# jumerckx/Monodepth2.jl

Measured on AMD Instinct MI355X. Metric: train-step images/sec, ResNet-18 416×128; 1/2/4/8 MI355X + roofline %, higher is better.
Workload: dtype fp32; 1 GPU; train_step resnet18 depth+pose decoders, 4-scale photometric loss, ADAM; batch_per_gpu=12, global_batch=12, height=128, width=416, parallelism=dp1

## Files before the change

monodepth2.jl_amd/csrc/model.cpp:

```cpp
#include "model.h"
#include "head.h"
#include "testmode.h"

#include <algorithm>
#include <cmath>
#include <cstring>

namespace md2 {

namespace {

struct PConv {
  int cin = 0, cout = 0, k = 1, stride = 1, pad = 0, reflect = 0;
  bool bias = false;
  long w = -1, b = -1;
};
struct PBN {
  int c = 0;
  long g = -1, b = -1;
};
struct BlockSpec {
  std::vector<PConv> convs;
  std::vector<PBN> bns;
  bool down = false;
// ... 600 lines not shown
      MD2_TRY(alloc(&pose_rep, 2L * ND * 6));
      MD2_TRY(alloc(&d_pose_rep, 2L * ND * 6));
      if (cfg.automask) MD2_TRY(alloc(&amask_rep, (long)ND * cfg.H * cfg.W));
    }
    tail.N = ND;
    tail.C = C;
    tail.W = cfg.W;
    tail.H = cfg.H;
    tail.nscales = A.nlevels;
    int li = 0;
    for (auto& d : br)
      if (d.head >= 0) {
        tail.dw[li] = 2 * d.w;
        tail.dh[li] = 2 * d.h;
        tail.smooth_w[li] = cfg.smoothness * cfg.scales[li];
        ++li;
      }
    tail.divisor = (float)A.nlevels;
    tail.smooth_normalize = 1;
    std::memcpy(tail.K, cfg.K, sizeof(tail.K));
    std::memcpy(tail.invK, cfg.invK, sizeof(tail.invK));
    tail.min_depth = cfg.min_depth;
    tail.max_depth = cfg.max_depth;
    tail.x_frame_stride = (long)C * cfg.H * cfg.W;
    tail.x_sample_stride = E > 0 ? 0 : 3 * tail.x_frame_stride;
    tail.target = cfg.target;
    tail.src0 = cfg.src0;
    tail.src1 = cfg.src1;
    tail.invert_mask = (cfg.src0 < cfg.target ? 1 : 0) | (cfg.src1 < cfg.target ? 2 : 0);
    tail.sigmoid_grad = 1;
    {
      float* q;
      MD2_TRY(alloc(&q, loss_tail_workspace_bytes(tail) / sizeof(float) + 64));
      tail_ws = q;
    }
    MD2_TRY(alloc(&loss_buf, 16));
    if (cfg.automask) MD2_TRY(alloc(&amask, (long)N * cfg.H * cfg.W));
    return build_pack_table();
  }

  struct ProfRec {
    hipEvent_t a, b;
    int cat;
    double work;
    char tag[64];
  };
  bool prof = false;
  std::vector<ProfRec> recs;
  std::vector<hipEvent_t> evpool;
  size_t evi = 0;
  hipEvent_t ev() {
    if (evi == evpool.size()) {
      hipEvent_t e;
      (void)hipEventCreate(&e);
      evpool.push_back(e);
    }
    return evpool[evi++];
  }
  hipEvent_t prof_begin(hipStream_t st) {
    if (!prof) return nullptr;
    hipEvent_t e = ev();
    (void)hipEventRecord(e, st);
    return e;
  }
  void prof_end(hipEvent_t a, int cat, double work, hipStream_t st, const char* pass = nullptr,
                const ConvShape* s = nullptr) {
    if (!prof) return;
    hipEvent_t b = ev();
    (void)hipEventRecord(b, st);
    ProfRec r{a, b, cat, work, {0}};
    if (pass && s) {
      const int ar = conv_last_arith();
      snprintf(r.tag, sizeof(r.tag), "%s %dx%d/%d%s %d->%d %dx%d n%d [%s]", pass, s->KH, s->KW, s->stride,
               s->reflect ? "r" : "", s->Cin, s->Cout, s->H, s->W, s->N,
               ar == 6 ? "bf16x6" : ar == 1 ? "fp32" : "valu");
    }
    else if (pass)
      snprintf(r.tag, sizeof(r.tag), "%s", pass);
    recs.push_back(r);
  }
  static double conv_flops(const ConvShape& s) {
    return 2.0 * s.N * (double)s.Ho * s.Wo * s.Cout * weight_cin(s) * s.KH * s.KW;
  }

  int conv_f(RConv& c, int nimg, const TensorIn& in, float* out, long out_bs, int act,
             int accumulate, hipStream_t st) {
    ConvShape s = c.s;
    s.N = nimg;
    TensorOut o;
    o.p0 = out;
    o.bs0 = out_bs;
    o.bias = P(c.p.b);
    o.act = act;
    o.accumulate = accumulate;
    hipEvent_t e = prof_begin(st);
    MD2_TRY(conv_fwd(s, in, c.wpf, o, ws_conv(), st));
    prof_end(e, c.cat, conv_flops(s), st, "fwd", &s);
    return MD2_OK;
  }
  int conv_f_bn(RConv& c, int nimg, const TensorIn& in, float* y, long out_bs, RBN& bn, long HW,
                hipStream_t st, int slot = 0) {
    ConvShape s = c.s;
    s.N = nimg;
    TensorOut o;
    o.p0 = y;
    o.bs0 = out_bs;
    o.bias = P(c.p.b);
    SplitKDefer d;
    BNStatsWs wst = bn_ws(bn, nimg, HW, slot);
    if (fuse_bnstats) d.stats = wst.partials;
    d.keep_reduce = !fuse_splitk;
    hipEvent_t e = prof_begin(st);
    MD2_TRY(conv_fwd(s, in, c.wpf, o, ws_conv(), st, fuse_splitk || fuse_bnstats ? &d : nullptr));
    if (d.stats_parts > 0) {
      if (bn_collapse) {
        MD2_CHECK_ARG(bn.p.c <= 4096, "conv_f_bn: BN channels");
        double* col = bn_collapsed + (long)slot * 2 * 4096;
        MD2_TRY(bn_partials_collapse(wst.partials, bn.p.c, d.stats_parts, col, st));
        bn.part = col;
        bn.parts = 1;
      } else {
        bn.part = wst.partials;
        bn.parts = d.stats_parts;
      }
      prof_end(e, c.cat, conv_flops(s), st, "fwd", &s);
      return MD2_OK;
    }
    if (d.splits > 0) {
      BNStatsWs w = bn_ws(bn, nimg, HW, slot);
      MD2_TRY(bn_stats_partial_slabs(SlabIn{d.slab, d.splits}, y, nimg, bn.p.c, HW, w, st));
      prof_end(e, c.cat, conv_flops(s), st, "fwd", &s);
      return MD2_OK;
    }
    prof_end(e, c.cat, conv_flops(s), st, "fwd", &s);
    return bn_fwd(bn, y, nimg, HW, st, slot);
  }
  const bool fuse_skip_bwd = [] {
    const char* v = getenv("MD2_FUSE_SKIP_BWD");
    return !(v && v[0] == '0');
  }();
  const bool fuse_pool_fwd = [] {
    const char* v = getenv("MD2_FUSE_POOL_FWD");
    return !(v && v[0] == '0');
  }();
  const bool fuse_pool_bwd = [] {
    const char* v = getenv("MD2_FUSE_POOL_BWD");
    return !(v && v[0] == '0');
  }();
  const bool bn_collapse = tuning_knob("MD2_BN_COLLAPSE", 0) != 0;
  const bool fuse_bnstats = [] {
    const char* v = getenv("MD2_FUSE_BNSTATS");
    return !(v && v[0] == '0');
  }();
  const bool fuse_splitk = [] {
    const char* v = getenv("MD2_FUSE_SPLITK");
    return !(v && v[0] == '0');
  }();
  static TensorIn tin(const float* p, int C, long HW) {
    TensorIn t;
    t.p0 = p;
    t.c0 = C;
    t.bs0 = (long)C * HW;
    return t;
  }

  PackJob* pack_jobs = nullptr;
  int pack_njobs = 0;
  long pack_blocks = 0;

  int build_pack_table() {
    std::vector<PackJob> jobs;
    auto pk = [&](RConv& c) { jobs.push_back(conv_pack_job(c.s, params + c.p.w, c.wpf, c.wpd)); };
    pk(stem);
    for (auto& sg : stages)
      for (auto& b : sg) {
        for (auto& e : b.st) pk(e.conv);
        if (b.down) pk(b.dconv);
      }
    for (auto& d : br) {
      pk(d.c1);
      pk(d.c2);
      if (d.head >= 0) pk(d.hc);
    }
    pk(sq);
    pk(p1);
    pk(p2);
    long blocks = 0;
    for (auto& j : jobs) {
      j.block_begin = blocks;
      blocks += conv_pack_job_blocks(j);
    }
    void* q = nullptr;
    MD2_HIP(hipMalloc(&q, jobs.size() * sizeof(PackJob)));
    allocs.push_back(q);
    MD2_HIP(hipMemcpy(q, jobs.data(), jobs.size() * sizeof(PackJob), hipMemcpyHostToDevice));
    pack_jobs = (PackJob*)q;
    pack_njobs = (int)jobs.size();
    pack_blocks = blocks;
    for (int k = 0; k < 6; ++k) {
      long b0, e0;
      segment_range(k, b0, e0);
      std::vector<PackJob> sj;
      long sb = 0;
      for (PackJob j : jobs) {
        const long off = (long)(j.w - params);
        if (off < b0 || off >= e0) continue;
        j.block_begin = sb;
        sb += conv_pack_job_blocks(j);
        sj.push_back(j);
      }
      seg_pack[k] = SegPack{};
      if (sj.empty()) continue;
      void* qs = nullptr;
      MD2_HIP(hipMalloc(&qs, sj.size() * sizeof(PackJob)));
      allocs.push_back(qs);
      MD2_HIP(hipMemcpy(qs, sj.data(), sj.size() * sizeof(PackJob), hipMemcpyHostToDevice));
      seg_pack[k] = SegPack{(PackJob*)qs, (int)sj.size(), sb};
    }
    return MD2_OK;
  }

  void segment_range(int k, long& b, long& e) const {
    const ArchSpec& S = spec;
    switch (k) {
      case 0: b = S.depth_begin; e = S.total; break;
      case 1: b = S.stage_begin[4]; e = S.depth_begin; break;
      case 2: b = S.stage_begin[3]; e = S.stage_begin[4]; break;
      case 3: b = S.stage_begin[2]; e = S.stage_begin[3]; break;
      case 4: b = S.stage_begin[1]; e = S.stage_begin[2]; break;
      default: b = 0; e = S.stage_begin[1]; break;
    }
  }

  int adam_segment(int k, float* am, float* av, float lr, float b1, float b2, float eps, float bc1,
                   float bc2, float gscale, hipStream_t st) {
    long b0, e0;
    segment_range(k, b0, e0);
    MD2_HIP(hipEventRecord(seg_ev, st));
    MD2_HIP(hipStreamWaitEvent(upd, seg_ev, 0));
    MD2_TRY(adam_step(params + b0, grads + b0, am + b0, av + b0, e0 - b0, lr, b1, b2, eps, bc1, bc2,
                      gscale, upd));
    if (seg_pack[k].njobs) MD2_TRY(conv_pack_batch(seg_pack[k].jobs, seg_pack[k].njobs, seg_pack[k].blocks, upd));
    MD2_HIP(hipEventRecord(upd_ev, upd));
    upd_recorded = true;
    return MD2_OK;
  }
  int adam_join(hipStream_t st) {
    if (upd_recorded) MD2_HIP(hipStreamWaitEvent(st, upd_ev, 0));
    return MD2_OK;
  }

  int repack(hipStream_t st) { return conv_pack_batch(pack_jobs, pack_njobs, pack_blocks, st); }

  BNStatsWs bn_ws(RBN& bn, int nimg, long HW, int slot) {
    BNStatsWs w = bnws;
    w.partials += slot * bn_slot;
    w.parts = bn_parts(bn.p.c, nimg, HW);
    bn.part = w.partials;
    bn.parts = w.parts;
    return w;
  }
  int bn_fwd(RBN& bn, const float* y, int nimg, long HW, hipStream_t st, int slot = 0) {
    return bn_stats_partial(y, nimg, bn.p.c, HW, bn_ws(bn, nimg, HW, slot), st);
  }
  BNStatsIn bn_in(const RBN& bn) {
    BNStatsIn s;
    s.part = bn.part;
    s.parts = bn.parts;
    s.gamma = P(bn.p.g);
    s.beta = P(bn.p.b);
    s.mean = bn.mean;
    s.invstd = bn.invstd;
    s.run_mean = bn.rmean;
    s.run_var = bn.rvar;
    return s;
  }

  bool testmode = false;
  float* wfold = nullptr;
  float* tm_st = nullptr;
  FoldJob* fold_jobs = nullptr;
  int fold_njobs = 0;
  long fold_blocks = 0;
  PackJob* tm_pack_jobs = nullptr;
  int tm_pack_njobs = 0;
  long tm_pack_blocks = 0;

  int testmode_alloc() {
    if (wfold) return MD2_OK;
    MD2_TRY(alloc(&wfold, spec.depth_begin));
    MD2_TRY(alloc(&tm_st, bn_layout.off[bn_layout.n]));
    std::vector<FoldJob> fj;
    std::vector<PackJob> pj;
    int k = 0;
    auto job = [&](RConv* c, RBN& bn) -> int {
      bn.ts = tm_st + bn_layout.off[k++];
      bn.tt = bn.ts + bn.p.c;
      FoldJob j;
      j.gamma = P(bn.p.g); j.beta = P(bn.p.b);
      j.mean = bn.rmean; j.var = bn.rvar;
      j.s = bn.ts; j.t = bn.tt;
      j.Cout = bn.p.c;
      if (c) {
        const long per = (long)c->p.cin * c->p.k * c->p.k;
        MD2_CHECK_ARG(per % 4 == 0 && c->p.cout == bn.p.c, "test mode: conv weight rows of 4n floats");
        j.w = params + c->p.w;
// ... 254 lines not shown
    MD2_TRY(conv_f(p2, 2 * N, tin(pc1, 256, hw4), pc2, 256 * hw4, ACT_RELU, 0, st));
    return pose_head_fwd(pc2, 2 * N, 256, hw4, P(spec.p3.w), P(spec.p3.b), means, pose, st);
  }

  int forward(const float* x, hipStream_t st) {
    const long fs = (long)cfg.arch.in_ch * cfg.H * cfg.W;
    TensorIn in;
    in.p0 = x;
    in.c0 = cfg.arch.in_ch;
    in.bdiv = N;
    in.bs0 = 3 * fs;
    in.bhi = fs;
    MD2_TRY(encoder(in, B, st));
    if (pose_overlap()) {
      MD2_TRY(stream_wait(st, side, fork_ev));
      MD2_TRY(pose_fwd(side));
      MD2_TRY(decoder_fwd(N, T0, st));
      MD2_TRY(stream_wait(side, st, join_ev));
    } else {
      MD2_TRY(decoder_fwd(N, T0, st));
      MD2_TRY(pose_fwd(st));
    }
    return MD2_OK;
  }

  int forward_loss(const float* x, const float* automask, float* loss, float* terms,
                   hipStream_t st) {
    MD2_TRY(forward(x, st));
    const float* disps[MAX_SCALES] = {};
    LossTailOut o{};
    int li = 0;
    for (auto& d : br)
      if (d.head >= 0) {
        disps[li] = d.disp;
        o.d_disp[li] = d.d_head;
        ++li;
      }
    o.loss = loss ? loss : loss_buf;
    o.terms = terms;
    o.d_pose = E > 0 ? d_pose_rep : d_pose;
    hipEvent_t pev[2 * MAX_SCALES] = {};
    if (prof) {
      for (int k = 0; k < 2; ++k) pev[k] = ev();
      o.photo_events = pev;
    }
    if (cfg.automask && !automask) {
      MD2_TRY(launch_automask(x, tail.x_sample_stride, tail.x_frame_stride, tail.target, tail.src0,
                              tail.src1, N, cfg.arch.in_ch, cfg.H, cfg.W, amask, st));
      automask = amask;
    }
    const float* tail_pose = pose;
    if (E > 0) {
      MD2_TRY(repeat_rows(pose, 2L * N, 6, NP, pose_rep, st));
      tail_pose = pose_rep;
      if (cfg.automask) {
        MD2_TRY(repeat_rows(automask, N, cfg.H * cfg.W, NP, amask_rep, st));
        automask = amask_rep;
      }
    }
    MD2_TRY(loss_tail_run(tail, disps, tail_pose, x, cfg.automask ? automask : nullptr, 1.f, o, tail_ws, st));
    if (E > 0) MD2_TRY(repeat_rows_adjoint(d_pose_rep, 2L * N, 6, NP, d_pose, st));
    if (prof) {
      const double bytes = (double)tail.nscales * ND * cfg.H * cfg.W * (8.0 + 12.0 * cfg.arch.in_ch);
      recs.push_back({pev[0], pev[1], PROF_PHOTO, bytes, "photometric (all scales)"});
    }
    return MD2_OK;
  }

  int profile_records(int max, double* ms, double* work, int* cat, char* tags, int tag_len,
                      int* count) {
    int k = 0;
    for (auto& r : recs) {
      if (k >= max) break;
      MD2_HIP(hipEventSynchronize(r.b));
      float t = 0.f;
      MD2_HIP(hipEventElapsedTime(&t, r.a, r.b));
      ms[k] = t;
      work[k] = r.work;
      cat[k] = r.cat;
      if (tags && tag_len > 0) {
        strncpy(tags + (long)k * tag_len, r.tag, tag_len - 1);
        tags[(long)k * tag_len + tag_len - 1] = 0;
      }
      ++k;
    }
    *count = k;
    recs.clear();
    evi = 0;
    return MD2_OK;
  }

  int profile_read(double* out, int ncat) {
    for (int c = 0; c < ncat * 3; ++c) out[c] = 0.0;
    for (auto& r : recs) {
      MD2_HIP(hipEventSynchronize(r.b));
      float ms = 0.f;
      MD2_HIP(hipEventElapsedTime(&ms, r.a, r.b));
      if (r.cat < ncat) {
        out[r.cat * 3 + 0] += ms;
        out[r.cat * 3 + 1] += r.work;
        out[r.cat * 3 + 2] += 1.0;
      }
    }
    recs.clear();
    evi = 0;
    return MD2_OK;
  }

  int conv_w(RConv& c, int nimg, const TensorIn& in, const float* dy, hipStream_t st) {
    ConvShape s = c.s;
    s.N = nimg;
    hipEvent_t e = prof_begin(st);
    MD2_TRY(conv_wgrad(s, in, dy, grads + c.p.w, Gd(c.p.b), 0, ws_conv(), st, c.p.b >= 0 ? bp_pending : nullptr,
                       bp_parts));
    bp_pending = nullptr;
    prof_end(e, c.cat, conv_flops(s), st, "wgrad", &s);
    return MD2_OK;
  }
  int conv_wd(RConv& c, int nimg, const TensorIn& in, const float* dy, float* dx, long dx_bs,
              int acc, hipStream_t st, float* dx1 = nullptr, long dx1_bs = 0, int c0 = 1 << 30) {
    MD2_TRY(conv_w(c, nimg, in, dy, st));
    return conv_d(c, nimg, dy, dx, dx_bs, acc, st, dx1, dx1_bs, c0);
  }
  int conv_d(RConv& c, int nimg, const float* dy, float* dx, long dx_bs, int acc, hipStream_t st,
             float* dx1 = nullptr, long dx1_bs = 0, int c0 = 1 << 30) {
    ConvShape s = c.s;
    s.N = nimg;
    TensorOut o;
    o.p0 = dx;
    o.bs0 = dx_bs;
    o.p1 = dx1;
    o.bs1 = dx1_bs;
    o.c0 = c0;
    o.accumulate = acc;
    hipEvent_t e = prof_begin(st);
    MD2_TRY(conv_dgrad(s, dy, c.wpd, o, ws_conv(), st));
    prof_end(e, c.cat, conv_flops(s), st, "dgrad", &s);
    return MD2_OK;
  }
  int conv_d_bn(RConv& c, int nimg, const float* dy, float* da, long da_bs, RBN& bn, const float* y,
                long HW, float* dyprev, hipStream_t st) {
    ConvShape s = c.s;
    s.N = nimg;
    TensorOut o;
    o.p0 = da;
    o.bs0 = da_bs;
    SplitKDefer d;
    hipEvent_t e = prof_begin(st);
    MD2_TRY(conv_dgrad(s, dy, c.wpd, o, ws_conv(), st, fuse_splitk ? &d : nullptr));
    if (d.splits == 0) {
      prof_end(e, c.cat, conv_flops(s), st, "dgrad", &s);
      return bn_bwd(bn, da, nullptr, y, nimg, HW, dyprev, nullptr, 0, st, true);
    }
    BNStatsWs w = bnws;
    w.parts = bn_parts(bn.p.c, nimg, HW);
    MD2_TRY(bn_bwd_partial_slabs(SlabIn{d.slab, d.splits}, da, y, bn.mean, bn.invstd, nimg, bn.p.c,
                                 HW, w, st, P(bn.p.g), P(bn.p.b)));
    prof_end(e, c.cat, conv_flops(s), st, "dgrad", &s);
    return bn_bwd_apply_fused(da, nullptr, y, bn.mean, bn.invstd, P(bn.p.g), w, Gd(bn.p.g),
                              Gd(bn.p.b), nimg, bn.p.c, HW, dyprev, nullptr, 0, st, P(bn.p.b));
  }
  float* bp_ws = nullptr;
  const float* bp_pending = nullptr;
  int bp_parts = 0;
  int act_bias(const float* out, const float* dout, float* dpre, int nimg, int C, long HW, int act,
               hipStream_t st, float* bp_buf = nullptr) {
    if (HW % 4 != 0 || (long)C * act_bias_parts(C, nimg, HW) > BP_WS) {
      bp_pending = nullptr;
      return act_backward(out, dout, dpre, (long)nimg * C * HW, act, st);
    }
    float* bp = bp_buf ? bp_buf : ws_bp();
    MD2_TRY(act_backward_bias(out, dout, dpre, nimg, C, HW, act, bp, st));
    bp_pending = bp;
    bp_parts = act_bias_parts(C, nimg, HW);
    return MD2_OK;
  }
  static constexpr long BP_WS = 8192;

  int bn_bwd(RBN& bn, const float* dout, const float* mask, const float* y, int nimg, long HW,
             float* dy, float* dres, int dres_acc, hipStream_t st, bool relu_from_y = false,
             SkipAdd sk = SkipAdd{}, int slot = 0) {
    BNStatsWs w = bnws;
    w.partials += slot * bn_slot;
    w.parts = bn_parts(bn.p.c, nimg, HW);
    const float* mg = relu_from_y ? P(bn.p.g) : nullptr;
    const float* mb = relu_from_y ? P(bn.p.b) : nullptr;
    if (relu_from_y) mask = nullptr;
    MD2_TRY(bn_bwd_partial(dout, mask, y, bn.mean, bn.invstd, nimg, bn.p.c, HW, w, st, mg, mb, sk));
    return bn_bwd_apply_fused(dout, mask, y, bn.mean, bn.invstd, P(bn.p.g), w, Gd(bn.p.g),
                              Gd(bn.p.b), nimg, bn.p.c, HW, dy, dres, dres_acc, st, mb, sk);
  }
  bool skip_fused(int si) const {
    return fuse_skip_bwd && si >= 1 && si <= 3 && d_skip[si] && ((long)featH[si] * featW[si]) % 4 == 0;
  }
  SkipAdd skip_add(int si) const {
    SkipAdd sk;
    if (!skip_fused(si)) return sk;
    const long fsz = (long)featC[si] * featH[si] * featW[si];
    sk.skip = d_skip[si];
    sk.lo = (long)T0 * fsz;
    sk.hi = (long)(T0 + N) * fsz;
    return sk;
  }

  int block_bwd(EncBlock& b, hipStream_t st, SkipAdd sk = SkipAdd{}, bool eov = false) {
    const int nimg = B;
    const long ohw = (long)b.H * b.W, ihw = (long)b.Hin * b.Win;
    const int ns = (int)b.st.size();
    EncStage& last = b.st.back();
    MD2_TRY(y_claim(ycur, st));
    MD2_TRY(bn_bwd(last.bn, b.d_out, last.a, last.y, nimg, ohw, ybuf(ycur), b.down ? G : b.d_in, 0, st,
                   false, sk));
    const bool dov = b.down && down_overlap();
    if (b.down) {
      hipStream_t sd = dov ? side : st;
      if (dov) MD2_TRY(stream_wait(st, side, fork_ev));
      MD2_TRY(bn_bwd(b.dbn, G, nullptr, b.yd, nimg, ohw, DYD, nullptr, 0, sd, false, SkipAdd{}, 1));
      side_ws = true;
      const int rc = conv_wd(b.dconv, nimg, tin(b.in, b.Cin, ihw), DYD, b.d_in, (long)b.Cin * ihw, 0, sd);
      side_ws = false;
      MD2_TRY(rc);
      if (dov) MD2_HIP(hipEventRecord(join_ev, side));
    }
    for (int k = ns - 1; k >= 0; --k) {
      EncStage& e = b.st[k];
      const float* xin = k == 0 ? b.in : b.st[k - 1].a;
      const int cin = e.conv.p.cin;
      const long hin = (long)e.conv.s.H * e.conv.s.W;
      float* dy = ybuf(ycur);
      const bool wmain = eov && k == 0 && enc_wgrad_main0;
      if (eov && !wmain) {
        MD2_TRY(stream_wait(st, side, fork_ev));
        side_ws = true;
        const int rc = conv_w(e.conv, nimg, tin(xin, cin, hin), dy, side);
        side_ws = false;
        MD2_TRY(rc);
        MD2_HIP(hipEventRecord(ev_y[ycur], side));
        y_pending[ycur] = true;
      } else if (!wmain) {
        MD2_TRY(conv_w(e.conv, nimg, tin(xin, cin, hin), dy, st));
      }
      if (k > 0) {
        EncStage& pe = b.st[k - 1];
        const int nx = ycur ^ 1;
        MD2_TRY(y_claim(nx, st));
        MD2_TRY(conv_d_bn(e.conv, nimg, dy, DA, (long)cin * hin, pe.bn, pe.y, hin, ybuf(nx), st));
        ycur = nx;
      } else {
        if (dov) MD2_HIP(hipStreamWaitEvent(st, join_ev, 0));
        MD2_TRY(conv_d(e.conv, nimg, dy, b.d_in, (long)cin * hin, 1, st));
        if (wmain) MD2_TRY(conv_w(e.conv, nimg, tin(xin, cin, hin), dy, st));
      }
    }
    return MD2_OK;
  }

  int pose_bwd(hipStream_t st) {
    side_ws = true;
    const int rc = pose_bwd_body(st);
    side_ws = false;
    return rc;
  }
  int pose_bwd_body(hipStream_t st) {
    const long hw4 = (long)featH[4] * featW[4];
    float* DP = DPRE_side;
    MD2_TRY(pose_head_bwd(d_pose, 2 * N, 256, hw4, P(spec.p3.w), means, DP, Gd(spec.p3.w),
                          Gd(spec.p3.b), st));
    MD2_TRY(act_bias(pc2, DP, DP, 2 * N, 256, hw4, ACT_RELU, st));
    MD2_TRY(conv_wd(p2, 2 * N, tin(pc1, 256, hw4), DP, d_pc1, 256 * hw4, 0, st));
    MD2_TRY(act_bias(pc1, d_pc1, d_pc1, 2 * N, 256, hw4, ACT_RELU, st));
    MD2_TRY(conv_wd(p1, 2 * N, pose_pairs_in(hw4), d_pc1, d_pin, 512 * hw4, 0, st));
    MD2_TRY(pair_grad_gather(d_pin, N, 256, hw4, pa, pb, d_sq, st));
    MD2_TRY(act_bias(sqo, d_sq, d_sq, B, 256, hw4, ACT_RELU, st));
    float* d_f4 = stages[3].back().d_out;
    return conv_wd(sq, B, tin(feat[4], featC[4], hw4), d_sq, d_f4, (long)featC[4] * hw4, 0, st);
  }

  int seg_decoder(hipStream_t st) {
    const bool ov = pose_overlap();
    if (ov) {
      MD2_TRY(stream_wait(st, side, fork_ev));
      MD2_TRY(pose_bwd(side));
      MD2_HIP(hipEventRecord(join_ev, side));
    } else {
      MD2_TRY(pose_bwd(st));
    }
    float* d_f4 = stages[3].back().d_out;
    const int nb = (int)br.size();
    {
      HeadJob jobs[MAX_HEADS];
      const int nh = head_jobs(jobs, ND);
      hipEvent_t e = prof_begin(st);
      MD2_TRY(heads_bwd(jobs, nh, hws, heads_bwd_workspace(jobs, nh) + 256, st));
      prof_end(e, PROF_CONV_OTHER, 2.0 * heads_flops(ND), st, "heads bwd");
    }
    const bool wov = wgrad_overlap();
    auto wgrad_side = [&](RConv& c, const TensorIn& in, const float* dy, hipEvent_t ready,
                          hipEvent_t done) -> int {
      MD2_TRY(stream_wait(st, side, ready));
      side_ws = true;
      const int rc = conv_w(c, ND, in, dy, side);
      side_ws = false;
      MD2_TRY(rc);
      MD2_HIP(hipEventRecord(done, side));
      return MD2_OK;
    };
    for (int i = nb - 1; i >= 0; --i) {
      DecBranch& d = br[i];
      const long hw = (long)d.h * d.w, hw2 = 4 * hw;
      const int co = d.b.cout;
      float* const dpre = DPRE;
      float* const do1 = DO1;
      const hipEvent_t evc2 = ev_c2, evc1 = ev_c1;
      float* const bpc2 = bp_dec[0];
      float* const bpc1 = bp_dec[1];
      if (wov && i < nb - 1) MD2_HIP(hipStreamWaitEvent(st, evc2, 0));
      MD2_TRY(act_bias(d.o2, d.d_o2, dpre, ND, co, hw2, ACT_ELU, st, wov ? bpc2 : nullptr));
      TensorIn in = tin(d.up, co, hw2);
      float* dskip = nullptr;
      long skip_bs = 0;
      if (d.b.cskip > 0) {
        const int fi = 4 - d.b.bid;
        if (E > 0) {
          in.p1 = emb_in[fi];
          in.bs1 = (long)(featC[fi] + Ep) * hw2;
          dskip = d_emb[fi];
          skip_bs = (long)(featC[fi] + Ep) * hw2;
        } else {
          in.p1 = feat[fi] + (long)T0 * featC[fi] * hw2;
          in.bs1 = (long)featC[fi] * hw2;
          dskip = d_skip[fi];
          skip_bs = (long)featC[fi] * hw2;
        }
      }
      if (wov) {
        MD2_TRY(wgrad_side(d.c2, in, dpre, ev_a, evc2));
        MD2_TRY(conv_d(d.c2, ND, dpre, DUP, co * hw2, 0, st, dskip, skip_bs, co));
      } else {
        MD2_TRY(conv_wd(d.c2, ND, in, dpre, DUP, co * hw2, 0, st, dskip, skip_bs, co));
      }
// ... 556 lines not shown
```

monodepth2.jl_amd/csrc/nn.h:

```cpp
#pragma once
#include "common.h"

namespace md2 {

struct BNStatsWs {
  double* partials;
  int parts;
};
int bn_parts(int C, long N, long HW);
struct SlabIn {
  const float* slab = nullptr;
  int splits = 0;
};
struct SkipAdd {
  const float* skip = nullptr;
  long lo = 0, hi = 0;
};
struct SkipSrc {
  const float* skip = nullptr;
  uint32_t skip_lo = 0, skip_hi = 0;
};
int bn_stats(const float* y, int N, int C, long HW, float eps, float momentum, float* mean,
             float* invstd, float* run_mean, float* run_var, BNStatsWs ws, hipStream_t st);
struct BNApply {
  const float* y; const float* mean; const float* invstd; const float* gamma; const float* beta;
  const float* y2 = nullptr; const float* mean2 = nullptr; const float* invstd2 = nullptr;
  const float* gamma2 = nullptr; const float* beta2 = nullptr;
  const float* res = nullptr;
  int relu = 0;
};
int bn_apply(const BNApply& p, float* out, int N, int C, long HW, hipStream_t st);

struct BNStatsIn {
  const double* part = nullptr;
  int parts = 0;
  float eps = 1e-5f, momentum = 0.1f;
  const float* gamma = nullptr; const float* beta = nullptr;
  float* mean = nullptr; float* invstd = nullptr;
  float* run_mean = nullptr; float* run_var = nullptr;
};
struct BNApplyFused {
  const float* y = nullptr; BNStatsIn s1;
  const float* y2 = nullptr; BNStatsIn s2;
  const float* res = nullptr;
  int relu = 0;
};
int bn_stats_partial(const float* y, int N, int C, long HW, BNStatsWs ws, hipStream_t st);
int bn_partials_collapse(const double* part, int C, int parts, double* out, hipStream_t st);
int bn_stats_partial_slabs(SlabIn sl, float* y, int N, int C, long HW, BNStatsWs ws, hipStream_t st);
int bn_apply_fused(const BNApplyFused& p, float* out, int N, int C, long HW, hipStream_t st);
int bn_bwd_reduce(const float* dout, const float* mask_out, const float* y, const float* mean,
                  const float* invstd, int N, int C, long HW, float* dgamma, float* dbeta,
                  BNStatsWs ws, hipStream_t st);
int bn_bwd_partial(const float* dout, const float* mask_out, const float* y, const float* mean,
                   const float* invstd, int N, int C, long HW, BNStatsWs ws, hipStream_t st,
                   const float* mgamma = nullptr, const float* mbeta = nullptr, SkipAdd sk = SkipAdd{});
int bn_bwd_partial_slabs(SlabIn sl, float* dout, const float* y, const float* mean,
                         const float* invstd, int N, int C, long HW, BNStatsWs ws, hipStream_t st,
                         const float* mgamma, const float* mbeta);
int bn_bwd_apply_fused(const float* dout, const float* mask_out, const float* y, const float* mean,
                       const float* invstd, const float* gamma, BNStatsWs ws, float* dgamma,
                       float* dbeta, int N, int C, long HW, float* dy, float* dres,
                       int dres_accumulate, hipStream_t st, const float* mbeta = nullptr,
                       SkipAdd sk = SkipAdd{});
int bn_bwd_apply(const float* dout, const float* mask_out, const float* y, const float* mean,
                 const float* invstd, const float* gamma, const float* dgamma,
                 const float* dbeta, int N, int C, long HW, float* dy, float* dres,
                 int dres_accumulate, hipStream_t st);

int bn_relu_maxpool(const BNApplyFused& p, float* act, int N, int C, int H, int W, float* y,
                    unsigned char* arg, int Ho, int Wo, hipStream_t st);
int maxpool_fwd(const float* x, int N, int C, int H, int W, float* y, unsigned char* arg,
                int Ho, int Wo, hipStream_t st);
int maxpool_bwd(const float* dy, const unsigned char* arg, int N, int C, int H, int W, int Ho,
                int Wo, float* dx, hipStream_t st, SkipAdd skip = SkipAdd{});

int upsample2_fwd(const float* x, int N, int C, int h, int w, float* y, hipStream_t st);
int upsample2_bwd(const float* dy, int N, int C, int h, int w, float* dx, hipStream_t st);
int mpi_embed_features(const float* feat, long sample_stride, int N, int C, int h, int w,
                       const float* bins, int P, int L, float* out, hipStream_t st, int Ctot = 0);
int plane_sum(const float* in, int N, int P, int Cin, int C, long hw, float* out, int accumulate,
              hipStream_t st);
int repeat_rows(const float* src, long rows, int cols, int P, float* dst, hipStream_t st);
int repeat_rows_adjoint(const float* src, long rows, int cols, int P, float* dst, hipStream_t st);
int concat_channels(const float* a, int ca, const float* b, int cb, int N, long hw, float* out,
                    hipStream_t st);

int pose_head_fwd(const float* x, int Q, int C, long HW, const float* w, const float* b,
                  float* means, float* pose, hipStream_t st);
int pose_head_bwd(const float* dpose, int Q, int C, long HW, const float* w, const float* means,
                  float* dx, float* dw, float* db, hipStream_t st);

int axpy(float* y, const float* x, long n, hipStream_t st);
int pair_gather(const float* sq, int N, int C, long HW, const int a[2], const int b[2], float* pin,
                hipStream_t st);
int pair_grad_gather(const float* dpin, int N, int C, long HW, const int a[2], const int b[2],
                     float* dsq, hipStream_t st);

int scale_inplace(float* x, long n, float s, hipStream_t st);
int sigmoid_cotangent(const float* g, const float* s, float* out, long n, hipStream_t st);
int flip_taps(const float* src, float* dst, long planes, int kh, int kw, hipStream_t st);
int adam_prep(int* step, float* bc, float b1, float b2, hipStream_t st);
int set_device_int(int* p, int v, hipStream_t st);
int adam_step_dev(float* p, const float* g, float* m, float* v, long n, float lr, float b1, float b2,
                  float eps, const float* bc, float gscale, hipStream_t st);
int adam_step(float* p, const float* g, float* m, float* v, long n, float lr, float b1, float b2,
              float eps, float bc1, float bc2, float gscale, hipStream_t st);

}
```

monodepth2.jl_amd/csrc/nn.hip:

```cpp
#include "nn.h"

namespace md2 {

int bn_parts(int C, long N, long HW) {
  long total = N * HW;
  int parts = (int)std::max(1L, std::min(1024L / std::max(1, C) + 1, total / 2048 + 1));
  return (int)std::min<long>(std::min(parts, 256), std::max(1L, N));
}

static FastDiv fd(long d) { return make_fastdiv((uint32_t)d); }
static int check_u31(long n) {
  MD2_CHECK_ARG(n >= 0 && n < (1L << 31), "tensor larger than 2^31 elements");
  return MD2_OK;
}

constexpr int BN_INFLIGHT = 4;

template <bool VEC, bool SLAB = false>
__global__ __launch_bounds__(256) void bn_stats_partial_kernel(const float* __restrict__ y, int C,
                                                               int HW, int N, int parts,
                                                               FastDiv fdu, double* __restrict__ part,
                                                               SlabIn sl = SlabIn{},
                                                               float* __restrict__ yout = nullptr) {
  __shared__ double red[8];
// ... 630 lines not shown
    hipLaunchKernelGGL(bn_bwd_apply_kernel<false>, dim3(cdiv(n, 256)), dim3(256), 0, st, dout,
                       mask_out, y, mean, invstd, gamma, dgamma, dbeta, (uint32_t)n, fd(HW), fd(C),
                       invL, dy, dres, dres_accumulate);
  MD2_LAUNCH_CHECK();
  return MD2_OK;
}


template <bool VEC, bool SKIP = false, int UPT = 1>
__global__ __launch_bounds__(256) void bn_bwd_apply_fused_kernel(
    const float* __restrict__ dout, const float* __restrict__ mask, const float* __restrict__ y,
    const float* __restrict__ mean, const float* __restrict__ invstd,
    const float* __restrict__ gamma, const double* __restrict__ part, int parts,
    float* __restrict__ dgamma, float* __restrict__ dbeta, uint32_t nu, FastDiv fdU, FastDiv fdC,
    float invL, float* __restrict__ dy, float* __restrict__ dres, int dres_acc,
    const float* __restrict__ mbeta, SkipSrc pd = SkipSrc{}) {
  static_assert(!SKIP || VEC, "SKIP: float4 units of a read dout");
  static_assert(VEC || UPT == 1, "scalar units: one per thread");
  __shared__ float s_k0[256], s_db[256], s_dg[256], s_mu[256], s_is[256], s_msc[256], s_msh[256];
  const uint32_t u0 = blockIdx.x * (256u * UPT);
  const uint32_t pl0 = fdiv(u0, fdU);
  const uint32_t npl = fdiv(min(u0 + 256u * UPT - 1u, nu - 1u), fdU) - pl0 + 1u;
  for (uint32_t t = threadIdx.x >> 6; t < npl; t += 4) {
    const uint32_t pl = pl0 + t;
    const int c = (int)(pl - fdiv(pl, fdC) * fdC.d);
    double sg = 0.0, sgx = 0.0;
    const double* q = part + (long)c * parts * 2;
    for (int p = threadIdx.x & 63; p < parts; p += 64) {
      sg += q[2 * p];
      sgx += q[2 * p + 1];
    }
    sg = wave_sum_d(sg);
    sgx = wave_sum_d(sgx);
    if ((threadIdx.x & 63) == 0) {
      const float dbf = (float)sg, dgf = (float)sgx;
      if (pl < fdC.d && pl * fdU.d >= u0) {
        dbeta[c] = dbf;
        dgamma[c] = dgf;
      }
      const float is = invstd[c];
      s_k0[t] = gamma[c] * is;
      s_db[t] = dbf * invL;
      s_dg[t] = dgf * invL;
      s_mu[t] = mean[c];
      s_is[t] = is;
      const YMask ym = ymask(gamma, mbeta, c, mean[c], is);
      s_msc[t] = ym.sc;
      s_msh[t] = ym.sh;
    }
  }
  __syncthreads();
  if (VEC) {
    float4 t[UPT], mv[UPT], v[UPT], qd[UPT];
#pragma unroll
    for (int j = 0; j < UPT; ++j) {
      const uint32_t u = u0 + threadIdx.x + 256u * j;
      const long i = 4L * (u < nu ? u : 0u);
      t[j] = *reinterpret_cast<const float4*>(dout + i);
      if (SKIP) t[j] = add_skip4(pd, (uint32_t)i, t[j]);
      if (mask) mv[j] = *reinterpret_cast<const float4*>(mask + i);
      v[j] = *reinterpret_cast<const float4*>(y + i);
      if (dres && dres_acc) qd[j] = *reinterpret_cast<const float4*>(dres + i);
    }
#pragma unroll
    for (int j = 0; j < UPT; ++j) {
      const uint32_t u = u0 + threadIdx.x + 256u * j;
      if (u >= nu) break;
      const long i = 4L * u;
      const uint32_t li = fdiv(u, fdU) - pl0;
      const float k0 = s_k0[li], db = s_db[li], dg = s_dg[li], mu = s_mu[li], is = s_is[li];
      const YMask ym{s_msc[li], s_msh[li], mbeta != nullptr};
      float g[4] = {t[j].x, t[j].y, t[j].z, t[j].w};
      if (mask) {
        const float4 m = mv[j];
        if (!(m.x > 0.f)) g[0] = 0.f;
        if (!(m.y > 0.f)) g[1] = 0.f;
        if (!(m.z > 0.f)) g[2] = 0.f;
        if (!(m.w > 0.f)) g[3] = 0.f;
      }
      const float yv[4] = {v[j].x, v[j].y, v[j].z, v[j].w};
#pragma unroll
      for (int k = 0; k < 4; ++k) g[k] = ymasked(g[k], yv[k], ym);
      float r[4];
#pragma unroll
      for (int k = 0; k < 4; ++k) r[k] = k0 * (g[k] - db - (yv[k] - mu) * is * dg);
      *reinterpret_cast<float4*>(dy + i) = make_float4(r[0], r[1], r[2], r[3]);
      if (dres) {
        float4 o = make_float4(g[0], g[1], g[2], g[3]);
        if (dres_acc) {
          const float4 q = qd[j];
          o.x += q.x; o.y += q.y; o.z += q.z; o.w += q.w;
        }
        *reinterpret_cast<float4*>(dres + i) = o;
      }
    }
  } else {
    const uint32_t u = u0 + threadIdx.x;
    if (u >= nu) return;
    const uint32_t li = fdiv(u, fdU) - pl0;
    const float k0 = s_k0[li], db = s_db[li], dg = s_dg[li], mu = s_mu[li], is = s_is[li];
    const YMask ym{s_msc[li], s_msh[li], mbeta != nullptr};
    float g = dout[u];
    if (mask && !(mask[u] > 0.f)) g = 0.f;
    g = ymasked(g, y[u], ym);
    const float xh = (y[u] - mu) * is;
    dy[u] = k0 * (g - db - xh * dg);
    if (dres) {
      if (dres_acc)
        dres[u] += g;
      else
        dres[u] = g;
    }
  }
}

int bn_bwd_apply_fused(const float* dout, const float* mask_out, const float* y, const float* mean,
                       const float* invstd, const float* gamma, BNStatsWs ws, float* dgamma,
                       float* dbeta, int N, int C, long HW, float* dy, float* dres,
                       int dres_accumulate, hipStream_t st, const float* mbeta, SkipAdd sk) {
  const long n = (long)N * C * HW;
  MD2_TRY(check_u31(n));
  MD2_CHECK_ARG(ws.partials && ws.parts >= 1, "bn_bwd_apply_fused: missing partials");
  MD2_CHECK_ARG(!sk.skip || (HW % 4 == 0 && sk.lo >= 0 && sk.lo <= sk.hi && sk.hi <= n),
                "bn_bwd: skip range / HW % 4");
  const float invL = 1.f / (float)((long)N * HW);
  if (HW % 4 == 0) {
    const long nu = n / 4;
    const int upt = bn_upt(nu, HW / 4);
    const dim3 grid(cdiv(nu, 256L * upt));
#define MD2_BWDA(SK, U)                                                                              \
  hipLaunchKernelGGL((bn_bwd_apply_fused_kernel<true, SK, U>), grid, dim3(256), 0, st, dout, mask_out, y, \
                     mean, invstd, gamma, ws.partials, ws.parts, dgamma, dbeta, (uint32_t)nu, fd(HW / 4), \
                     fd(C), invL, dy, dres, dres_accumulate, mbeta, skip_src(sk))
    if (sk.skip) {
      if (upt == 8) MD2_BWDA(true, 8);
      else if (upt == 4) MD2_BWDA(true, 4);
      else if (upt == 2) MD2_BWDA(true, 2);
      else MD2_BWDA(true, 1);
    } else {
      if (upt == 8) MD2_BWDA(false, 8);
      else if (upt == 4) MD2_BWDA(false, 4);
      else if (upt == 2) MD2_BWDA(false, 2);
      else MD2_BWDA(false, 1);
    }
#undef MD2_BWDA
  } else
    hipLaunchKernelGGL(bn_bwd_apply_fused_kernel<false>, dim3(cdiv(n, 256)), dim3(256), 0, st,
                       dout, mask_out, y, mean, invstd, gamma, ws.partials, ws.parts, dgamma, dbeta,
                       (uint32_t)n, fd(HW), fd(C), invL, dy, dres, dres_accumulate, mbeta);
  MD2_LAUNCH_CHECK();
  return MD2_OK;
}

template <bool EVENW>
__global__ __launch_bounds__(256) void maxpool_fwd_kernel(const float* __restrict__ x, int H, int W,
                                                          float* __restrict__ y,
                                                          unsigned char* __restrict__ arg, int Ho,
                                                          FastDiv fdWo, FastDiv fdHo, uint32_t n) {
  const uint32_t i = blockIdx.x * 256 + threadIdx.x;
  if (i >= n) return;
  const uint32_t r = fdiv(i, fdWo), plane = fdiv(r, fdHo);
  const int ow = (int)(i - r * fdWo.d), oh = (int)(r - plane * fdHo.d);
  const float* p = x + plane * (uint32_t)(H * W);
  float best = -INFINITY;
  int bi = 0;
  const int iw = ow * 2;
#pragma unroll
  for (int kh = 0; kh < 3; ++kh) {
    const int ih = oh * 2 - 1 + kh;
    if (ih < 0 || ih >= H) continue;
    const float* row = p + ih * W;
    float v0 = -INFINITY, v1, v2 = -INFINITY;
    if (iw > 0) v0 = row[iw - 1];
    if (EVENW) {
      const float2 t = *reinterpret_cast<const float2*>(row + iw);
      v1 = t.x;
      v2 = t.y;
    } else {
      v1 = row[iw];
      if (iw + 1 < W) v2 = row[iw + 1];
    }
    if (v0 > best) { best = v0; bi = kh * 3; }
    if (v1 > best) { best = v1; bi = kh * 3 + 1; }
    if (v2 > best) { best = v2; bi = kh * 3 + 2; }
  }
  y[i] = best;
  arg[i] = (unsigned char)bi;
}

template <bool EVENW, bool SKIP = false>
__global__ __launch_bounds__(256) void maxpool_bwd_kernel(const float* __restrict__ dy,
                                                          const unsigned char* __restrict__ arg,
                                                          int H, int W, int Ho, FastDiv fdWo,
                                                          FastDiv fdHo, float* __restrict__ dx,
                                                          uint32_t n, SkipSrc sk = SkipSrc{}) {
  static_assert(!SKIP || EVENW, "SKIP: even width");
  const uint32_t t = blockIdx.x * 256 + threadIdx.x;
  if (t >= n) return;
  const uint32_t r = fdiv(t, fdWo), plane = fdiv(r, fdHo);
  const int Wo = (int)fdWo.d;
  const int j = (int)(t - r * fdWo.d), i = (int)(r - plane * fdHo.d);
  const bool hasr = i + 1 < Ho, hasc = j + 1 < Wo;
  const uint32_t o = t;
  const int a00 = arg[o];
  const float g00 = dy[o];
  int a01 = -1, a10 = -1, a11 = -1;
  float g01 = 0.f, g10 = 0.f, g11 = 0.f;
  if (hasc) { a01 = arg[o + 1]; g01 = dy[o + 1]; }
  if (hasr) { a10 = arg[o + Wo]; g10 = dy[o + Wo]; }
  if (hasr && hasc) { a11 = arg[o + Wo + 1]; g11 = dy[o + Wo + 1]; }
  const float e00 = a00 == 4 ? g00 : 0.f;
  const float e01 = (a00 == 5 ? g00 : 0.f) + (a01 == 3 ? g01 : 0.f);
  const float e10 = (a00 == 7 ? g00 : 0.f) + (a10 == 1 ? g10 : 0.f);
  const float e11 = (a00 == 8 ? g00 : 0.f) + (a01 == 6 ? g01 : 0.f) + (a10 == 2 ? g10 : 0.f) +
                    (a11 == 0 ? g11 : 0.f);
  const uint32_t qi = plane * (uint32_t)(H * W) + (2 * i) * W + 2 * j;
  float* q = dx + qi;
  if (EVENW) {
    float2 r0 = make_float2(e00, e01), r1 = make_float2(e10, e11);
    if (SKIP && qi >= sk.skip_lo && qi < sk.skip_hi) {
      const float2 k0 = *reinterpret_cast<const float2*>(sk.skip + (qi - sk.skip_lo));
      r0.x += k0.x; r0.y += k0.y;
      if (2 * i + 1 < H) {
        const float2 k1 = *reinterpret_cast<const float2*>(sk.skip + (qi + W - sk.skip_lo));
        r1.x += k1.x; r1.y += k1.y;
      }
    }
    *reinterpret_cast<float2*>(q) = r0;
    if (2 * i + 1 < H) *reinterpret_cast<float2*>(q + W) = r1;
  } else {
    q[0] = e00;
    if (2 * j + 1 < W) q[1] = e01;
    if (2 * i + 1 < H) {
      q[W] = e10;
      if (2 * j + 1 < W) q[W + 1] = e11;
    }
  }
}

__global__ __launch_bounds__(256) void bn_relu_maxpool_kernel(BNApplyFused p, float* __restrict__ act,
                                                              int H, int W, float* __restrict__ y,
                                                              unsigned char* __restrict__ arg,
                                                              FastDiv fdWo, FastDiv fdHo, FastDiv fdU,
                                                              FastDiv fdC, uint32_t n, double total) {
  __shared__ float s_sc[256], s_sh[256];
  const uint32_t u0 = blockIdx.x * 256u;
  const uint32_t pl0 = fdiv(u0, fdU);
  const uint32_t npl = fdiv(min(u0 + 255u, n - 1u), fdU) - pl0 + 1u;
  for (uint32_t t = threadIdx.x >> 6; t < npl; t += 4) {
    const uint32_t pl = pl0 + t;
    const int c = (int)(pl - fdiv(pl, fdC) * fdC.d);
    const bool owner = pl < fdC.d && pl * fdU.d >= u0;
    float sc, sh;
    bn_finalise_plane(p.s1, c, total, owner, sc, sh);
    if ((threadIdx.x & 63) == 0) {
      s_sc[t] = sc;
      s_sh[t] = sh;
    }
  }
  __syncthreads();
  const uint32_t i = u0 + threadIdx.x;
  if (i >= n) return;
  const uint32_t r = fdiv(i, fdWo), plane = fdiv(r, fdHo);
  const int ow = (int)(i - r * fdWo.d), oh = (int)(r - plane * fdHo.d);
  const float sc = s_sc[plane - pl0], sh = s_sh[plane - pl0];
  const uint32_t base = plane * (uint32_t)(H * W);
  const float* src = p.y + base;
  float best = -INFINITY;
  int bi = 0;
  const int iw = ow * 2;
#pragma unroll
  for (int kh = 0; kh < 3; ++kh) {
    const int ih = oh * 2 - 1 + kh;
    if (ih < 0) continue;
    const float* row = src + ih * W;
    float v0 = -INFINITY;
    if (iw > 0) v0 = fmaxf(__fmaf_rn(row[iw - 1], sc, sh), 0.f);
    const float2 t = *reinterpret_cast<const float2*>(row + iw);
    const float v1 = fmaxf(__fmaf_rn(t.x, sc, sh), 0.f);
    const float v2 = fmaxf(__fmaf_rn(t.y, sc, sh), 0.f);
    if (kh > 0) *reinterpret_cast<float2*>(act + base + ih * W + iw) = make_float2(v1, v2);
    if (v0 > best) { best = v0; bi = kh * 3; }
    if (v1 > best) { best = v1; bi = kh * 3 + 1; }
    if (v2 > best) { best = v2; bi = kh * 3 + 2; }
  }
  y[i] = best;
  arg[i] = (unsigned char)bi;
}

int bn_relu_maxpool(const BNApplyFused& p, float* act, int N, int C, int H, int W, float* y,
                    unsigned char* arg, int Ho, int Wo, hipStream_t st) {
  MD2_CHECK_ARG(H % 2 == 0 && W % 2 == 0 && Ho == H / 2 && Wo == W / 2,
                "bn_relu_maxpool: even input, 3x3/2 pad-1 output shape");
  MD2_CHECK_ARG(p.y && p.s1.part && p.s1.parts >= 1 && !p.y2 && !p.res && p.relu,
                "bn_relu_maxpool: BN+ReLU without residual / second branch");
  const long n = (long)N * C * Ho * Wo;
  MD2_TRY(check_u31((long)N * C * H * W));
  const double total = (double)((long)N * H * W);
  hipLaunchKernelGGL(bn_relu_maxpool_kernel, dim3(cdiv(n, 256)), dim3(256), 0, st, p, act, H, W, y,
                     arg, fd(Wo), fd(Ho), fd((long)Ho * Wo), fd(C), (uint32_t)n, total);
  MD2_LAUNCH_CHECK();
  return MD2_OK;
}

int maxpool_fwd(const float* x, int N, int C, int H, int W, float* y, unsigned char* arg, int Ho,
                int Wo, hipStream_t st) {
// ... 603 lines not shown
```

Before: 1909 images/s.

## Fuse BN backward reduce and apply into one per-channel block kernel

Adds a single-kernel BatchNorm backward that runs one 1024-thread block per channel and keeps that channel's gradients and activations in registers. It reduces dbeta and dgamma in the block and then writes dy and the residual gradient directly, replacing the separate partial-reduce and apply kernels. The split-K dgrad slabs are also summed inside this kernel. It is used only when N*HW/4 fits in 2048 float4 units, so large-resolution layers keep the old two-kernel path. The trade-off is low parallelism for layers with few channels, since each channel becomes a single block.

```diff
diff --git a/monodepth2.jl_amd/csrc/model.cpp b/monodepth2.jl_amd/csrc/model.cpp
--- a/monodepth2.jl_amd/csrc/model.cpp
+++ b/monodepth2.jl_amd/csrc/model.cpp
@@ -776,6 +776,10 @@
     const char* v = getenv("MD2_FUSE_BNSTATS");
     return !(v && v[0] == '0');
   }();
+  const bool fuse_bn_bwd = [] {
+    const char* v = getenv("MD2_FUSE_BN_BWD");
+    return !(v && v[0] == '0');
+  }();
   const bool fuse_splitk = [] {
     const char* v = getenv("MD2_FUSE_SPLITK");
     return !(v && v[0] == '0');
@@ -1336,6 +1340,13 @@
       prof_end(e, c.cat, conv_flops(s), st, "dgrad", &s);
       return bn_bwd(bn, da, nullptr, y, nimg, HW, dyprev, nullptr, 0, st, true);
     }
+    if (fuse_bn_bwd && bn_bwd_channel_fits(nimg, HW)) {
+      MD2_TRY(bn_bwd_channel(nullptr, SlabIn{d.slab, d.splits}, nullptr, y, bn.mean, bn.invstd,
+                             P(bn.p.g), P(bn.p.b), Gd(bn.p.g), Gd(bn.p.b), nimg, bn.p.c, HW, dyprev,
+                             nullptr, 0, st));
+      prof_end(e, c.cat, conv_flops(s), st, "dgrad", &s);
+      return MD2_OK;
+    }
     BNStatsWs w = bnws;
     w.parts = bn_parts(bn.p.c, nimg, HW);
     MD2_TRY(bn_bwd_partial_slabs(SlabIn{d.slab, d.splits}, da, y, bn.mean, bn.invstd, nimg, bn.p.c,
@@ -1370,6 +1381,9 @@
     const float* mg = relu_from_y ? P(bn.p.g) : nullptr;
     const float* mb = relu_from_y ? P(bn.p.b) : nullptr;
     if (relu_from_y) mask = nullptr;
+    if (fuse_bn_bwd && bn_bwd_channel_fits(nimg, HW))
+      return bn_bwd_channel(dout, SlabIn{}, mask, y, bn.mean, bn.invstd, P(bn.p.g), mb, Gd(bn.p.g),
+                            Gd(bn.p.b), nimg, bn.p.c, HW, dy, dres, dres_acc, st, sk);
     MD2_TRY(bn_bwd_partial(dout, mask, y, bn.mean, bn.invstd, nimg, bn.p.c, HW, w, st, mg, mb, sk));
     return bn_bwd_apply_fused(dout, mask, y, bn.mean, bn.invstd, P(bn.p.g), w, Gd(bn.p.g),
                               Gd(bn.p.b), nimg, bn.p.c, HW, dy, dres, dres_acc, st, mb, sk);
diff --git a/monodepth2.jl_amd/csrc/nn.h b/monodepth2.jl_amd/csrc/nn.h
--- a/monodepth2.jl_amd/csrc/nn.h
+++ b/monodepth2.jl_amd/csrc/nn.h
@@ -63,6 +63,11 @@
                        float* dbeta, int N, int C, long HW, float* dy, float* dres,
                        int dres_accumulate, hipStream_t st, const float* mbeta = nullptr,
                        SkipAdd sk = SkipAdd{});
+bool bn_bwd_channel_fits(int N, long HW);
+int bn_bwd_channel(const float* dout, SlabIn sl, const float* mask_out, const float* y,
+                   const float* mean, const float* invstd, const float* gamma, const float* mbeta,
+                   float* dgamma, float* dbeta, int N, int C, long HW, float* dy, float* dres,
+                   int dres_accumulate, hipStream_t st, SkipAdd sk = SkipAdd{});
 int bn_bwd_apply(const float* dout, const float* mask_out, const float* y, const float* mean,
                  const float* invstd, const float* gamma, const float* dgamma,
                  const float* dbeta, int N, int C, long HW, float* dy, float* dres,
diff --git a/monodepth2.jl_amd/csrc/nn.hip b/monodepth2.jl_amd/csrc/nn.hip
--- a/monodepth2.jl_amd/csrc/nn.hip
+++ b/monodepth2.jl_amd/csrc/nn.hip
@@ -806,6 +806,148 @@
   return MD2_OK;
 }
 
+constexpr int BN_CH_THREADS = 1024;
+constexpr int BN_CH_UNITS = 2;
+
+template <bool SLAB, bool SKIP>
+__global__ __launch_bounds__(BN_CH_THREADS) void bn_bwd_channel_kernel(
+    const float* __restrict__ dout, const float* __restrict__ mask, const float* __restrict__ y,
+    const float* __restrict__ mean, const float* __restrict__ invstd,
+    const float* __restrict__ gamma, const float* __restrict__ mbeta, int C, int N, FastDiv fdu,
+    float invL, float* __restrict__ dgamma, float* __restrict__ dbeta, float* __restrict__ dy,
+    float* __restrict__ dres, int dres_acc, SlabIn sl, SkipSrc pd) {
+  static_assert(!(SLAB && SKIP), "SLAB: no skip addend (and no mask tensor)");
+  constexpr int NW = BN_CH_THREADS / 64;
+  __shared__ double red[2 * NW];
+  const int c = blockIdx.x;
+  const uint32_t U = fdu.d, HW = 4u * U, nu = (uint32_t)N * U;
+  const float mu = mean[c], is = invstd[c];
+  const YMask ym = ymask(gamma, mbeta, c, mu, is);
+  const long sstride = (long)C * N * HW;
+  float4 gv[BN_CH_UNITS], yv[BN_CH_UNITS];
+  uint32_t off[BN_CH_UNITS];
+#pragma unroll
+  for (int h = 0; h < BN_CH_UNITS; ++h) {
+    const uint32_t e = threadIdx.x + (uint32_t)BN_CH_THREADS * h;
+    gv[h] = yv[h] = make_float4(0.f, 0.f, 0.f, 0.f);
+    off[h] = 0;
+    if (e >= nu) continue;
+    const uint32_t im = fdiv(e, fdu), k = e - im * U;
+    const uint32_t i = (im * (uint32_t)C + (uint32_t)c) * HW + 4u * k;
+    off[h] = i;
+    if (!SLAB) gv[h] = *reinterpret_cast<const float4*>(dout + i);
+    if (SKIP) gv[h] = add_skip4(pd, i, gv[h]);
+    yv[h] = *reinterpret_cast<const float4*>(y + i);
+    if (mask) {
+      const float4 m = *reinterpret_cast<const float4*>(mask + i);
+      if (!(m.x > 0.f)) gv[h].x = 0.f;
+      if (!(m.y > 0.f)) gv[h].y = 0.f;
+      if (!(m.z > 0.f)) gv[h].z = 0.f;
+      if (!(m.w > 0.f)) gv[h].w = 0.f;
+    }
+  }
+  if (SLAB) {
+    const float* sq = sl.slab + (long)c * N * HW;
+    for (int q = 0; q < sl.splits; ++q, sq += sstride) {
+      float4 t[BN_CH_UNITS];
+#pragma unroll
+      for (int h = 0; h < BN_CH_UNITS; ++h) {
+        const uint32_t e = threadIdx.x + (uint32_t)BN_CH_THREADS * h;
+        if (e < nu) t[h] = *reinterpret_cast<const float4*>(sq + 4u * e);
+      }
+#pragma unroll
+      for (int h = 0; h < BN_CH_UNITS; ++h) {
+        if (threadIdx.x + (uint32_t)BN_CH_THREADS * h >= nu) continue;
+        gv[h].x += t[h].x; gv[h].y += t[h].y; gv[h].z += t[h].z; gv[h].w += t[h].w;
+      }
+    }
+  }
+  double sg = 0.0, sgx = 0.0;
+#pragma unroll
+  for (int h = 0; h < BN_CH_UNITS; ++h) {
+    if (threadIdx.x + (uint32_t)BN_CH_THREADS * h >= nu) continue;
+    float4& g = gv[h];
+    const float4 v = yv[h];
+    g.x = ymasked(g.x, v.x, ym);
+    g.y = ymasked(g.y, v.y, ym);
+    g.z = ymasked(g.z, v.z, ym);
+    g.w = ymasked(g.w, v.w, ym);
+    sg += (double)g.x + (double)g.y + (double)g.z + (double)g.w;
+    sgx += (double)g.x * (double)((v.x - mu) * is) + (double)g.y * (double)((v.y - mu) * is) +
+           (double)g.z * (double)((v.z - mu) * is) + (double)g.w * (double)((v.w - mu) * is);
+  }
+  sg = wave_sum_d(sg);
+  sgx = wave_sum_d(sgx);
+  const int lane = threadIdx.x & 63, wid = threadIdx.x >> 6;
+  if (lane == 0) {
+    red[wid] = sg;
+    red[NW + wid] = sgx;
+  }
+  __syncthreads();
+  double tg = red[0], tgx = red[NW];
+#pragma unroll
+  for (int w = 1; w < NW; ++w) {
+    tg += red[w];
+    tgx += red[NW + w];
+  }
+  const float dbf = (float)tg, dgf = (float)tgx;
+  if (threadIdx.x == 0) {
+    dbeta[c] = dbf;
+    dgamma[c] = dgf;
+  }
+  const float k0 = __fmul_rn(gamma[c], is), db = __fmul_rn(dbf, invL), dg = __fmul_rn(dgf, invL);
+#pragma unroll
+  for (int h = 0; h < BN_CH_UNITS; ++h) {
+    if (threadIdx.x + (uint32_t)BN_CH_THREADS * h >= nu) continue;
+    const uint32_t i = off[h];
+    const float g[4] = {gv[h].x, gv[h].y, gv[h].z, gv[h].w};
+    const float v[4] = {yv[h].x, yv[h].y, yv[h].z, yv[h].w};
+    float r[4];
+#pragma unroll
+    for (int k = 0; k < 4; ++k) {
+      const float xh = __fmul_rn(__fsub_rn(v[k], mu), is);
+      r[k] = __fmul_rn(k0, __fmaf_rn(-xh, dg, __fsub_rn(g[k], db)));
+    }
+    *reinterpret_cast<float4*>(dy + i) = make_float4(r[0], r[1], r[2], r[3]);
+    if (dres) {
+      float4 o = gv[h];
+      if (dres_acc) {
+        const float4 q = *reinterpret_cast<const float4*>(dres + i);
+        o.x += q.x; o.y += q.y; o.z += q.z; o.w += q.w;
+      }
+      *reinterpret_cast<float4*>(dres + i) = o;
+    }
+  }
+}
+
+bool bn_bwd_channel_fits(int N, long HW) {
+  return HW % 4 == 0 && (long)N * (HW / 4) <= (long)BN_CH_THREADS * BN_CH_UNITS;
+}
+
+int bn_bwd_channel(const float* dout, SlabIn sl, const float* mask_out, const float* y,
+                   const float* mean, const float* invstd, const float* gamma, const float* mbeta,
+                   float* dgamma, float* dbeta, int N, int C, long HW, float* dy, float* dres,
+                   int dres_accumulate, hipStream_t st, SkipAdd sk) {
+  const long n = (long)N * C * HW;
+  MD2_TRY(check_u31(n));
+  MD2_CHECK_ARG(bn_bwd_channel_fits(N, HW), "bn_bwd_channel: a channel must fit in a block");
+  MD2_CHECK_ARG((sl.slab != nullptr) != (dout != nullptr) &&
+                    (!sl.slab || (sl.splits >= 1 && !sk.skip && !mask_out)),
+                "bn_bwd_channel: dout or slabs (slabs without skip / mask tensor)");
+  MD2_CHECK_ARG(!sk.skip || (sk.lo >= 0 && sk.lo <= sk.hi && sk.hi <= n), "bn_bwd: skip range");
+  const float invL = 1.f / (float)((long)N * HW);
+#define MD2_BWDC(SL, SK)                                                                        \
+  hipLaunchKernelGGL((bn_bwd_channel_kernel<SL, SK>), dim3(C), dim3(BN_CH_THREADS), 0, st, dout, \
+                     mask_out, y, mean, invstd, gamma, mbeta, C, N, fd(HW / 4), invL, dgamma,    \
+                     dbeta, dy, dres, dres_accumulate, sl, skip_src(sk))
+  if (sl.slab) MD2_BWDC(true, false);
+  else if (sk.skip) MD2_BWDC(false, true);
+  else MD2_BWDC(false, false);
+#undef MD2_BWDC
+  MD2_LAUNCH_CHECK();
+  return MD2_OK;
+}
+
 template <bool EVENW>
 __global__ __launch_bounds__(256) void maxpool_fwd_kernel(const float* __restrict__ x, int H, int W,
                                                           float* __restrict__ y,
```

Result: faster. 1931 images/s, median of 6 (+1.1%).
